# YiZhangCUG/liblcg

Measured on AMD Instinct MI355X. Metric: cg_iterations_per_sec, higher is better.
Workload: dtype f64

## Files before the change

liblcg_amd/csrc/driver.hpp:

```cpp
#pragma once

#include <algorithm>
#include <chrono>
#include <cstdlib>
#include <functional>
#include <cstring>
#include <thread>
#include <typeinfo>
#include <vector>

#include "devcommon.hpp"

namespace lcgh {

#define TRY(x) do { int rc_ = (x); if (rc_) return rc_; } while (0)
inline uintptr_t al(const void *p) { return (uintptr_t)p; }
double global_rows_of(Ctx &c, int n, const void *afp, const void *inst);

template <class Op> int launch_vec(const Op &op, long n, bool cplx, uintptr_t align_or, double *partials, hipStream_t s)
{
    const bool v2 = !cplx && (align_or & 15) == 0;
    const int g = grid_for(v2 ? (n + 1) / 2 : n);
    if (v2) hipLaunchKernelGGL((k_vec<Op, true>), dim3(g), dim3(VB), 0, s, op, n, partials);
    else hipLaunchKernelGGL((k_vec<Op, false>), dim3(g), dim3(VB), 0, s, op, n, partials);
    return g;
}

struct Driver {
    Ctx &c;
    long n;
    bool cplx;
    int max_it, abs_diff;
    double eps;
    int enq = 0;
    bool user_cb = false;

    Driver(Ctx &c_, long n_, bool cplx_, int max_it_, double eps_, int abs_diff_)
        : c(c_), n(n_), cplx(cplx_), max_it(max_it_), abs_diff(abs_diff_), eps(eps_) {}
    ~Driver() { c.in_solve = false; }
    Driver(const Driver &) = delete;

    template <class Op> int vec(Op op, uintptr_t align_or = 0) { return vec_n(op, n, align_or); }
    template <class Op> int vec_rows(Op op, int row0, uintptr_t align_or)
    {
        const PartCount keep = pcnt;
        double *table = c.partials;
        c.partials = table + (size_t)row0 * MAXG;
        int rc = vec_n(op, n, align_or);
        c.partials = table;
        const int g = pcnt.g[0];
        pcnt = keep;
        for (int r = 0; r < Op::NR; r++) pcnt.g[row0 + r] = g;
        return rc;
    }
    template <class Op> int vec_n(Op op, long n, uintptr_t align_or)
    {
        c.cnt_vec++;
        op.st = c.state;
        const int g = launch_vec(op, n, cplx, align_or, c.partials, c.stream);
        if (Op::NR > 0) pcnt.all(g);
        HIPCHK(hipGetLastError());
        return dbg(typeid(Op).name());
    }
    template <class Fin, class Op> int vecf(Fin fin, Op op, uintptr_t align_or = 0)
    {
        if (comm_active()) {
            int rc = scal(fin);
            return rc ? rc : vec(op, align_or);
        }
        c.cnt_vec++;
        const bool v2 = !cplx && (align_or & 15) == 0;
        const int g = grid_for(v2 ? (n + 1) / 2 : n);
        DevState *cur = c.state, *next = c.state == c.state_pair[0] ? c.state_pair[1] : c.state_pair[0];
        double *pin = c.partials, *pout = c.partials == c.partials_pair[0] ? c.partials_pair[1] : c.partials_pair[0];
        if (v2) hipLaunchKernelGGL((k_vecf<Fin, Op, true>), dim3(g), dim3(VB), 0, c.stream, fin, op, n, pin, pcnt, pout, cur, next);
        else hipLaunchKernelGGL((k_vecf<Fin, Op, false>), dim3(g), dim3(VB), 0, c.stream, fin, op, n, pin, pcnt, pout, cur, next);
        HIPCHK(hipGetLastError());
        c.state = next;
        if (Op::NR > 0) { c.partials = pout; pcnt.all(g); }
        return dbg(typeid(Op).name());
    }
    PartCount pcnt = [] { PartCount p; p.all(1); return p; }();
    std::function<int()> tail;
    int run_tail() { if (!tail) return 0; auto t = std::move(tail); tail = nullptr; return t(); }
    bool debug_sync = debug_level() >= 2;
    int dbg(const char *what)
    {
        if (!debug_sync) return 0;
        std::fprintf(stderr, "[lcg_hip] %s ...", what); std::fflush(stderr);
        HIPCHK(hipStreamSynchronize(c.stream));
        std::fprintf(stderr, " ok\n");
        return 0;
    }

    DevState *snap_to = nullptr;
    int snap_taken = 0;
    template <class Fin> int scal(Fin fin)
    {
        const PartCount g = pcnt;
        XgBox xb;
        c.cnt_scal++;
        if (comm_active() && Fin::NR > 0) c.cnt_allreduce++;
        if (snap_to) snap_taken++;
        if (comm_active() && Fin::NR > 0 && xg_box(&xb)) {
            hipLaunchKernelGGL((k_scal<Fin>), dim3(1), dim3(VB), 0, c.stream, fin, c.partials, g, c.state, SC_XGMI, xb, snap_to);
        } else if (comm_active() && Fin::NR > 0) {
            hipLaunchKernelGGL((k_scal<Fin>), dim3(1), dim3(VB), 0, c.stream, fin, c.partials, g, c.state, SC_REDUCE, xb, (DevState *)nullptr);
            int rc = comm_allreduce(c.state->red, Fin::NR, c.stream);
            if (rc) return rc;
            hipLaunchKernelGGL((k_scal<Fin>), dim3(1), dim3(VB), 0, c.stream, fin, c.partials, g, c.state, SC_FIN, xb, snap_to);
        } else {
            hipLaunchKernelGGL((k_scal<Fin>), dim3(1), dim3(VB), 0, c.stream, fin, c.partials, g, c.state, SC_FUSED, xb, snap_to);
        }
        HIPCHK(hipGetLastError());
        return dbg(typeid(Fin).name());
    }

    int init_state(double n_global)
    {
        c.in_solve = true; c.ax_rc = 0; c.cnt_vec = c.cnt_scal = c.cnt_allreduce = c.cnt_ax = 0;
        DevState h;
        std::memset(&h, 0, sizeof h);
        h.eps = eps; h.abs_diff = abs_diff; h.n_global = n_global; h.host = c.hstat_dev;
        h.pub_mask = comm_active() ? 0x3fffffff : ((cplx ? 2 * n : n) >= (1 << 20) ? 0 : 3);
        c.hstat->it = 0; c.hstat->done = 0; c.hstat->status = 0; c.hstat->t = 0; c.hstat->residual = 0.0;
        (void)lcg_hip_last_ax_mean_us();
        *c.state_stage = h;
        HIPCHK(hipMemcpyAsync(c.state, c.state_stage, sizeof h, hipMemcpyHostToDevice, c.stream));
        HIPCHK(hipEventRecord(c.ev_a, c.stream));
        HIPCHK(hipStreamWaitEvent(c.comm_stream, c.ev_a, 0));
        return 0;
    }
    int read_state(DevState &h)
    {
        HIPCHK(hipMemcpyAsync(&h, c.state, sizeof h, hipMemcpyDeviceToHost, c.stream));
        HIPCHK(hipStreamSynchronize(c.stream));
        return 0;
    }

    template <class F> int timed_ax(F &&call)
    {
        c.cnt_ax++;
        if (c.profile && (c.ax_seq++ % c.profile_every) == 0 && c.prof_used + 2 <= (int)c.prof_ev.size()) {
            HIPCHK(hipEventRecord(c.prof_ev[c.prof_used], c.stream));
            call();
            HIPCHK(hipEventRecord(c.prof_ev[c.prof_used + 1], c.stream));
            c.prof_used += 2;
        } else {
            call();
        }
        return c.ax_rc;
    }
    template <class F> int checked_mx(F &&call) { call(); return c.ax_rc; }

    template <class Body, class Pfp>
    int run(Body &&body, bool has_pfp, Pfp &&pfp, int code_max_it, int code_nan)
    {
        DevState h;
        int rc = 0;
        if (has_pfp || user_cb) {
            rc = read_state(h);
            if (rc) return rc;
            if (h.status == ST_ALREADY) {
                if (has_pfp) pfp(h.residual, 0);
                finish(h);
                return LCG_ALREADY_OPTIMIZIED;
            }
        }
        if (has_pfp) {
            for (;;) {
                if (pfp(h.residual, h.t)) { finish(h); return LCG_STOP; }
                if (h.residual <= eps) { finish(h); return LCG_CONVERGENCE; }
                if (max_it > 0 && h.t + 1 > max_it) { finish(h); return code_max_it; }
                rc = body(); if (rc) return rc;
                enq++;
                rc = read_state(h); if (rc) return rc;
                if (h.status == ST_COMM) return comm_lost(h);
                if (h.status == ST_NAN) { finish(h); return code_nan; }
            }
        }
        if (comm_active()) return run_lockstep(body, code_max_it, code_nan);
        const long work = cplx ? 2 * n : n;
        const int inflight = work >= (1 << 20) ? 6 : 24;
        for (;;) {
            if (max_it > 0 && enq >= max_it) break;
            rc = body(); if (rc) return rc;
            enq++;
            if (c.hstat->done) break;
            int spins = 0;
            while (c.hstat->it < enq - inflight && !c.hstat->done) {
                if (++spins > 2000) { std::this_thread::sleep_for(std::chrono::microseconds(20)); }
                if (spins > 200000) {
                    rc = read_state(h); if (rc) return rc;
                    if (h.done || h.it >= enq - inflight) break;
                    spins = 0;
                }
            }
            if ((enq & 255) == 0) {
                rc = read_state(h); if (rc) return rc;
                if (h.done) break;
            }
        }
        rc = run_tail(); if (rc) return rc;
        rc = read_state(h); if (rc) return rc;
        if (h.status == ST_COMM) return comm_lost(h);
        finish(h);
        if (h.status == ST_ALREADY) return LCG_ALREADY_OPTIMIZIED;
        if (h.status == ST_NAN) return code_nan;
        if (h.done && h.status == ST_CONVERGED) return LCG_CONVERGENCE;
        return code_max_it;
    }

    template <class Body>
    int run_lockstep(Body &&body, int code_max_it, int code_nan)
    {
        constexpr int batch = 8;
        int nb = 0, rc = 0;
        DevState h;
        for (;;) {
            int todo = batch;
            if (max_it > 0) todo = std::min(batch, max_it - enq);
            if (todo <= 0) break;
            const int slot = nb & 1;
            for (int i = 0; i < todo; i++) {
                if (i == todo - 1) { snap_to = c.snap_dev[slot]; snap_taken = 0; }
                rc = body();
                if (rc) { snap_to = nullptr; return rc; }
                enq++;
            }
            snap_to = nullptr;
            if (!snap_taken) HIPCHK(hipMemcpyAsync(c.snap[slot], c.state, sizeof(DevState), hipMemcpyDeviceToHost, c.stream));
            HIPCHK(hipEventRecord(c.snap_ev[slot], c.stream));
            nb++;
            if (nb >= 2) {
                const int prev = (nb - 2) & 1;
                HIPCHK(hipEventSynchronize(c.snap_ev[prev]));
                if (c.snap[prev]->done) break;
            }
        }
        if (nb > 0) {
            HIPCHK(hipEventSynchronize(c.snap_ev[(nb - 1) & 1]));
            HIPCHK(hipStreamSynchronize(c.stream));
            std::memcpy(&h, c.snap[(nb - 1) & 1], sizeof h);
        } else {
            rc = read_state(h); if (rc) return rc;
        }
        if (h.status == ST_COMM) return comm_lost(h);
        finish(h);
        if (h.status == ST_ALREADY) return LCG_ALREADY_OPTIMIZIED;
        if (h.status == ST_NAN) return code_nan;
        if (h.done && h.status == ST_CONVERGED) return LCG_CONVERGENCE;
        return code_max_it;
    }

    int comm_lost(const DevState &h)
    {
        finish(h);
        c.err = "direct all-reduce: a peer's contribution did not arrive in time";
        return LCG_HIP_E_COMM;
    }

    void finish(const DevState &h)
    {
        c.last_iters = h.t;
        c.last_residual = h.residual;
        c.last_ax_calls = c.prof_used / 2;
        c.last_ax_mean_us = 0.0;
        c.prof_pending = c.profile ? c.prof_used : 0;
        c.prof_used = 0;
    }
};

struct HostBridge {
    double *dm = nullptr, *dB = nullptr;
    double *hm = nullptr;
    size_t bytes = 0;
    bool active = false;
    int open(int mem, double *&m, const double *&B, size_t nbytes, hipStream_t s)
    {
        if (mem == LCG_HIP_MEM_DEVICE) return 0;
        active = true; bytes = nbytes; hm = m;
        HIPCHK(hipMalloc(&dm, nbytes));
        HIPCHK(hipMalloc(&dB, nbytes));
        HIPCHK(hipMemcpyAsync(dm, m, nbytes, hipMemcpyHostToDevice, s));
        HIPCHK(hipMemcpyAsync(dB, B, nbytes, hipMemcpyHostToDevice, s));
        m = dm; B = dB;
        return 0;
    }
    int close(hipStream_t s)
// ... 317 lines not shown
```

liblcg_amd/csrc/solvers_real.hip:

```cpp
#include <functional>

#include "driver.hpp"

namespace lcgh {

constexpr int CG1_AUTO_ROWS = 1 << 20;


struct OpDot1 {
    static constexpr int NR = 1, SKIP = SKIP_DONE;
    DevState *st; const double *a, *b;
    __device__ void prep() {}
    template <class T> __device__ void apply(long i, double *acc) { acc[0] += dotp(ld<T>(a, i), ld<T>(b, i)); }
};
struct OpDot2 {
    static constexpr int NR = 2, SKIP = SKIP_DONE;
    DevState *st; const double *a, *b;
    __device__ void prep() {}
    template <class T> __device__ void apply(long i, double *acc)
    {
        const T x = ld<T>(a, i);
        acc[0] += dotp(x, ld<T>(b, i));
        acc[1] += dotp(x, x);
    }
};

struct FinAlpha {
    static constexpr int NR = 1;
    __device__ void operator()(DevState *st, const double *sum) const
    {
        st->it++;
        if (st->done) return;
        st->s[S_AK] = st->s[S_RHO] / sum[0];
    }
};
struct FinOmega {
    static constexpr int NR = 2;
    __device__ void operator()(DevState *st, const double *sum) const
    {
        if (st->done) return;
        st->s[S_WK] = sum[0] / sum[1];
    }
};

struct FinInit {
    static constexpr int NR = 3;
    __device__ void operator()(DevState *st, const double *sum) const
    {
        const double m2 = clamp1(sum[0]), g2 = sum[1];
        st->s[S_M2] = m2; st->s[S_G2] = g2; st->s[S_RHO] = sum[2];
        double r;
        bool already = false;
        if (st->abs_diff && sqrt(g2) / st->n_global <= st->eps) { r = sqrt(g2) / st->n_global; already = true; }
        else if (g2 / m2 <= st->eps) { r = g2 / m2; already = true; }
        else r = st->abs_diff ? sqrt(g2) / st->n_global : g2 / m2;
        st->residual = r;
        if (already) { st->done = 1; st->status = ST_ALREADY; }
        publish(st);
    }
};

template <bool BICG>
struct FinClose {
    static constexpr int NR = 4;
    __device__ void operator()(DevState *st, const double *sum) const
    {
        if (!st->done) {
            st->s[S_M2] = clamp1(sum[0]);
            if (sum[3] > 0.0 || sum[0] != sum[0]) {
                st->t++;
                st->done = 1; st->status = ST_NAN;
            } else {
                const double rho_new = sum[2];
                st->s[S_BK] = BICG ? (st->s[S_AK] / st->s[S_WK]) * rho_new / st->s[S_RHO]
                                   : rho_new / st->s[S_RHO];
                st->s[S_RHO] = rho_new;
                st->s[S_G2] = sum[1];
                st->t++;
                stop_rule(st, sum[1], st->s[S_M2]);
            }
        }
        publish(st);
    }
};

struct OpZeroProbe {
    static constexpr int NR = 1, SKIP = SKIP_NEVER;
    DevState *st; const double *m;
    __device__ void prep() {}
    template <class T> __device__ void apply(long i, double *acc) { acc[0] += nonzeros(ld<T>(m, i)); }
    static __device__ double nonzeros(double v) { return v != 0.0 ? 1.0 : 0.0; }
    static __device__ double nonzeros(double2 v) { return (v.x != 0.0 ? 1.0 : 0.0) + (v.y != 0.0 ? 1.0 : 0.0); }
};
struct FinZeroGuess {
    static constexpr int NR = 1;
    __device__ void operator()(DevState *st, const double *sum) const { st->zero_guess = sum[0] == 0.0 ? 1 : 0; }
};

struct OpCgInit {
    static constexpr int NR = 3, SKIP = SKIP_NEVER;
    DevState *st; const double *Ad, *B, *m; double *g, *d;
    double *clear = nullptr;
    bool zg = false;
    __device__ void prep() { zg = st->zero_guess != 0; }
    template <class T> __device__ void apply(long i, double *acc)
    {
        const T av = ldz<T>(Ad, i, zg);
        if (zg && clear) st_(clear, i, av);
        const T gv = vsub(av, ld<T>(B, i));
        const T mv = ldz<T>(m, i, zg);
        st_(g, i, gv); st_(d, i, vneg(gv));
        acc[0] += dotp(mv, mv);
        const double gg = dotp(gv, gv);
        acc[1] += gg; acc[2] += gg;
    }
};
struct OpCgUpdate {
    static constexpr int NR = 4, SKIP = SKIP_DONE;
    DevState *st; double *m, *g; const double *d, *Ad; double ak; bool nt = false;
    __device__ void prep() { ak = st->s[S_AK]; }
    template <class T> __device__ void apply(long i, double *acc)
    {
        const T mv = vadd(ldp<T>(m, i, nt), ak * ld<T>(d, i));
        const T gv = vadd(ld<T>(g, i), ak * ldp<T>(Ad, i, nt));
        stp(m, i, mv, nt); st_(g, i, gv);
        acc[0] += dotp(mv, mv);
        const double gg = dotp(gv, gv);
        acc[1] += gg; acc[2] += gg;
        acc[3] += nanflag(mv);
    }
};
struct OpCgDir {
    static constexpr int NR = 0, SKIP = SKIP_DIR;
    DevState *st; double *d; const double *g; double bk; bool nt = false;
    __device__ void prep() { bk = st->s[S_BK]; }
    template <class T> __device__ void apply(long i, double *)
    {
        st_(d, i, vsub(bk * ld<T>(d, i), ldp<T>(g, i, nt)));
    }
};

struct OpCg1UpdateSums {
    static constexpr int NR = 4, SKIP = SKIP_DONE;
    DevState *st; double *m, *g, *d, *Ad; const double *w; double ak, bk; bool nt = false;
    __device__ void prep() { ak = st->s[S_AK]; bk = st->s[S_BK]; }
    template <class T> __device__ void apply(long i, double *acc)
    {
        const T g0 = ld<T>(g, i);
        const T dv = vsub(bk * ldp<T>(d, i, nt), g0);
        const T sv = vsub(bk * ldp<T>(Ad, i, nt), ldp<T>(w, i, nt));
        stp(d, i, dv, nt); stp(Ad, i, sv, nt);
        const T mv = vadd(ldp<T>(m, i, nt), ak * dv);
        const T gv = vadd(g0, ak * sv);
        stp(m, i, mv, nt); st_(g, i, gv);
        acc[0] += dotp(mv, mv);
        acc[1] += dotp(gv, gv);
        acc[3] += nanflag(mv);
    }
};
struct FinCg1Start {
    static constexpr int NR = 1;
    __device__ void operator()(DevState *st, const double *sum) const
    {
        if (st->done) return;
        st->s[S_AK] = st->s[S_RHO] / sum[0];
        st->s[S_BK] = 0.0;
    }
};

struct OpResidual {
    static constexpr int NR = 0, SKIP = SKIP_NEVER;
    DevState *st; const double *Ax, *B; double *r;
    double *clear = nullptr;
    bool zg = false;
    __device__ void prep() { zg = st->zero_guess != 0; }
    template <class T> __device__ void apply(long i, double *)
    {
        const T av = ldz<T>(Ax, i, zg);
        if (zg && clear) st_(clear, i, av);
        st_(r, i, vsub(ld<T>(B, i), av));
    }
};
struct OpPcgInit2 {
    static constexpr int NR = 3, SKIP = SKIP_NEVER;
    DevState *st; const double *z, *m, *r; double *d;
    __device__ void prep() {}
    template <class T> __device__ void apply(long i, double *acc)
    {
        const T zv = ld<T>(z, i), mv = ld<T>(m, i), rv = ld<T>(r, i);
        st_(d, i, zv);
        acc[0] += dotp(mv, mv); acc[1] += dotp(rv, rv); acc[2] += dotp(zv, rv);
    }
};
struct OpPcgUpdate {
    static constexpr int NR = 0, SKIP = SKIP_DONE;
    DevState *st; double *m, *r; const double *d, *Ad; double ak;
    __device__ void prep() { ak = st->s[S_AK]; }
    template <class T> __device__ void apply(long i, double *)
    {
        st_(m, i, vadd(ld<T>(m, i), ak * ld<T>(d, i)));
        st_(r, i, vsub(ld<T>(r, i), ak * ld<T>(Ad, i)));
    }
};
struct OpPcgDots {
    static constexpr int NR = 4, SKIP = SKIP_DONE;
    DevState *st; const double *m, *r, *z;
    __device__ void prep() {}
    template <class T> __device__ void apply(long i, double *acc)
    {
        const T mv = ld<T>(m, i), rv = ld<T>(r, i), zv = ld<T>(z, i);
        acc[0] += dotp(mv, mv); acc[1] += dotp(rv, rv); acc[2] += dotp(zv, rv); acc[3] += nanflag(mv);
    }
};
struct OpPcgUpdateJacobi {
    static constexpr int NR = 4, SKIP = SKIP_DONE;
    DevState *st; double *m, *r, *z; const double *d, *Ad, *invdiag; double ak; bool nt = false;
    __device__ void prep() { ak = st->s[S_AK]; }
    template <class T> __device__ void apply(long i, double *acc)
    {
        const T mv = vadd(ldp<T>(m, i, nt), ak * ld<T>(d, i));
        const T rv = vsub(ld<T>(r, i), ak * ldp<T>(Ad, i, nt));
        const T zv = vmul(ldp<T>(invdiag, i, nt), rv);
        stp(m, i, mv, nt); st_(r, i, rv); st_(z, i, zv);
        acc[0] += dotp(mv, mv); acc[1] += dotp(rv, rv); acc[2] += dotp(zv, rv); acc[3] += nanflag(mv);
    }
};
struct OpPcgDir {
    static constexpr int NR = 0, SKIP = SKIP_DIR;
    DevState *st; double *d; const double *z; double bk; bool nt = false;
    __device__ void prep() { bk = st->s[S_BK]; }
    template <class T> __device__ void apply(long i, double *) { st_(d, i, vadd(ldp<T>(z, i, nt), bk * ld<T>(d, i))); }
};

struct OpPcg1UpdateSums {
    static constexpr int NR = 5, SKIP = SKIP_DONE;
    DevState *st; double *m, *r, *z, *d, *Ad; const double *w, *invdiag; double ak, bk;
    __device__ void prep() { ak = st->s[S_AK]; bk = st->s[S_BK]; }
    template <class T> __device__ void apply(long i, double *acc)
    {
        const T dv = vadd(ld<T>(z, i), bk * ld<T>(d, i));
        const T sv = vadd(ld<T>(w, i), bk * ld<T>(Ad, i));
        st_(d, i, dv); st_(Ad, i, sv);
        const T mv = vadd(ld<T>(m, i), ak * dv);
        const T rv = vsub(ld<T>(r, i), ak * sv);
        const T zv = vmul(ld<T>(invdiag, i), rv);
        st_(m, i, mv); st_(r, i, rv); st_(z, i, zv);
        acc[0] += dotp(mv, mv); acc[1] += dotp(rv, rv); acc[2] += dotp(zv, rv); acc[3] += nanflag(mv);
    }
};
struct FinPcg1Close {
    static constexpr int NR = 5;
    __device__ void operator()(DevState *st, const double *sum) const
    {
        st->it++;
        if (!st->done) {
            st->s[S_M2] = clamp1(sum[0]);
            if (sum[3] > 0.0 || sum[0] != sum[0]) {
                st->t++;
                st->done = 1; st->status = ST_NAN;
            } else {
                const double rho_new = sum[2];
                const double bk = rho_new / st->s[S_RHO];
                st->s[S_AK] = rho_new / (sum[4] - bk * rho_new / st->s[S_AK]);
                st->s[S_BK] = bk;
                st->s[S_RHO] = rho_new;
                st->s[S_G2] = sum[1];
                st->t++;
                stop_rule(st, sum[1], st->s[S_M2]);
            }
        }
        publish(st);
    }
};

template <bool WITH_U>
struct OpShadowInit {
    static constexpr int NR = 3, SKIP = SKIP_NEVER;
    DevState *st; const double *Ax, *B, *m; double *r, *r0, *p, *u; bool zg = false;
    __device__ void prep() { zg = st->zero_guess != 0; }
    template <class T> __device__ void apply(long i, double *acc)
    {
        const T rv = vsub(ld<T>(B, i), ldz<T>(Ax, i, zg));
        const T mv = ldz<T>(m, i, zg);
        st_(r, i, rv); st_(r0, i, rv); st_(p, i, rv);
        if (WITH_U) st_(u, i, rv);
        acc[0] += dotp(mv, mv);
        const double rr = dotp(rv, rv);
        acc[1] += rr; acc[2] += rr;
    }
};
struct OpCgsQW {
    static constexpr int NR = 0, SKIP = SKIP_DONE;
    DevState *st; const double *u, *Ax; double *q, *w; double ak; bool nt = false;
    __device__ void prep() { ak = st->s[S_AK]; }
    template <class T> __device__ void apply(long i, double *)
    {
        const T uv = ld<T>(u, i);
        const T qv = vsub(uv, ak * ld<T>(Ax, i));
        st_(q, i, qv); st_(w, i, vadd(uv, qv));
    }
};
struct OpCgsUpdate {
    static constexpr int NR = 4, SKIP = SKIP_DONE;
    DevState *st; double *m, *r; const double *w, *Ax, *r0; double ak; bool nt = false;
    __device__ void prep() { ak = st->s[S_AK]; }
    template <class T> __device__ void apply(long i, double *acc)
    {
        const T mv = vadd(ldp<T>(m, i, nt), ak * ld<T>(w, i));
        const T rv = vsub(ld<T>(r, i), ak * ld<T>(Ax, i));
        stp(m, i, mv, nt); st_(r, i, rv);
        acc[0] += dotp(mv, mv); acc[1] += dotp(rv, rv); acc[2] += dotp(rv, ld<T>(r0, i)); acc[3] += nanflag(mv);
    }
};
struct OpCgsDir {
    static constexpr int NR = 0, SKIP = SKIP_DIR;
    DevState *st; double *u, *p; const double *r, *q; double bk; bool nt = false;
    __device__ void prep() { bk = st->s[S_BK]; }
    template <class T> __device__ void apply(long i, double *)
    {
        const T qv = ld<T>(q, i);
        const T uv = vadd(ld<T>(r, i), bk * qv);
        st_(u, i, uv);
        st_(p, i, vadd(uv, bk * vadd(qv, bk * ld<T>(p, i))));
    }
};
struct OpBicgS {
    static constexpr int NR = 0, SKIP = SKIP_DONE;
    DevState *st; const double *r, *Ap; double *s; double ak; bool nt = false;
    __device__ void prep() { ak = st->s[S_AK]; }
    template <class T> __device__ void apply(long i, double *) { st_(s, i, vsub(ld<T>(r, i), ak * ld<T>(Ap, i))); }
};
struct OpBicgUpdate {
    static constexpr int NR = 4, SKIP = SKIP_DONE;
    DevState *st; double *m, *r; const double *p, *s, *Ax, *r0; double ak, wk; bool nt = false;
    __device__ void prep() { ak = st->s[S_AK]; wk = st->s[S_WK]; }
    template <class T> __device__ void apply(long i, double *acc)
    {
        const T sv = ld<T>(s, i);
        const T mv = vadd(ldp<T>(m, i, nt), vadd(ak * ld<T>(p, i), wk * sv));
        const T rv = vsub(sv, wk * ld<T>(Ax, i));
        stp(m, i, mv, nt); st_(r, i, rv);
        acc[0] += dotp(mv, mv); acc[1] += dotp(rv, rv); acc[2] += dotp(rv, ld<T>(r0, i)); acc[3] += nanflag(mv);
    }
};
struct OpBicgDir {
    static constexpr int NR = 0, SKIP = SKIP_DIR;
    DevState *st; double *p; const double *r, *Ap; double bk, wk; bool nt = false;
    __device__ void prep() { bk = st->s[S_BK]; wk = st->s[S_WK]; }
    template <class T> __device__ void apply(long i, double *)
    {
        st_(p, i, vadd(ld<T>(r, i), bk * vsub(ld<T>(p, i), wk * ld<T>(Ap, i))));
    }
};


static bool stream_vectors(long n, lcg_axfunc_ptr Afp, void *inst)
{
    static const int env = [] { const char *e = std::getenv("LCG_HIP_NT_VECTORS"); return e ? atoi(e) : -1; }();
    if (env >= 0) return env != 0;
    if (n * 40L <= (128L << 20)) return false;
    if (Afp == lcg_hip_csr_ax && inst != nullptr) {
        const lcg_hip_csr *A = static_cast<const lcg_hip_csr *>(inst);
        const long nnz = A->distributed ? (long)A->loc.nnz + (long)A->rem.nnz : (long)A->main.nnz;
        return nnz * 12L >= (512L << 20);
    }
    return n * 40L > (256L << 20);
}

struct RealSolve : Solve<false> {
    using Solve::Solve;
    int ax_setup(const double *m0, double *y)
    {
        if (Afp != lcg_hip_csr_ax || inst == nullptr) return ax(m0, y);
        int rc = drv.vec(OpZeroProbe{c.state, m0}, (uintptr_t)m0);
        if (!rc) rc = drv.scal(FinZeroGuess{});
        if (rc) return rc;
        c.ax_skip = &c.state->zero_guess;
        Afp(inst, m0, y, n);
        c.ax_skip = nullptr;
        return c.ax_rc;
    }
    int ax_dot(const double *x, double *y, const double *u, bool yy, int row, bool *fused)
    {
        int f = 0, slots = 0;
        const bool builtin = Afp == lcg_hip_csr_ax && inst != nullptr;
        int rc = drv.timed_ax([&] {
            if (builtin) f = csr_ax_dot(static_cast<lcg_hip_csr *>(inst), x, y, u, yy ? 1 : 0, c.ax_partials, &slots, c.stream, &c.state->done);
            if (f == 0) Afp(inst, x, y, n);
            else if (f < 0 && !c.ax_rc) c.ax_rc = f;
        });
        *fused = f == 1;
        if (f == 1) {
            PartCount &pc = drv.pcnt;
            pc.axp = c.ax_partials; pc.ax_n = slots; pc.ax_row = row; pc.ax_yy = yy ? 1 : 0;
            pc.g[row] = 0; if (yy) pc.g[row + 1] = 0;
        }
        return rc;
    }

    bool last_body(int row)
    {
        const bool last = para.max_iterations > 0 && drv.enq + 1 >= para.max_iterations;
        if (last) { drv.pcnt.ax_n = 0; drv.pcnt.ax_row = -1; drv.pcnt.g[row] = 0; }
        return last;
    }
    template <class Close, class Op, class Rest>
    int run_self_closing(const Op &upd, uintptr_t align_or, Rest &&rest)
    {
        bool first = true;
        drv.tail = [&]() -> int { return first ? drv.scal(FinCg1Start{}) : drv.scal(Close{}); };
        const int rc = run_loop([&]() -> int {
            TRY(first ? drv.vecf(FinCg1Start{}, upd, align_or) : drv.vecf(Close{}, upd, align_or));
            first = false;
            return rest();
        });
        drv.tail = nullptr;
        return rc;
    }
};

static int check_args(const lcg_para &p, int n, const double *m, const double *B)
{
    if (n <= 0) return LCG_INVILAD_VARIABLE_SIZE;
    if (p.max_iterations < 0) return LCG_INVILAD_MAX_ITERATIONS;
    if (p.epsilon <= 0.0 || p.epsilon >= 1.0) return LCG_INVILAD_EPSILON;
    if (m == nullptr || B == nullptr) return LCG_INVALID_POINTER;
    return 0;
}

static int solve_cg(lcg_axfunc_ptr Afp, lcg_progress_ptr Pfp, double *m, const double *B, int n,
                    const lcg_para *param, void *inst, double *Gk, double *Dk, double *ADk, int mem)
{
    const lcg_para p = param ? *param : lcg_hip_default_parameters();
    TRY(check_args(p, n, m, B));
    TRY(ensure_init());
    RealSolve k(p, n, inst, Afp, Pfp);
    Ctx &c = k.c;
    TRY(k.open(mem, m, B));
    double *g, *d, *Ad;
    TRY(k.get(g, Gk)); TRY(k.get(d, Dk)); TRY(k.get(Ad, ADk));
    const bool one_reduction = c.cg_schedule == LCG_HIP_CG_ONE_REDUCTION ||
                               (c.cg_schedule == LCG_HIP_CG_AUTO && (comm_active() || (n < CG1_AUTO_ROWS && Afp == lcg_hip_csr_ax)));
    double *w = nullptr;
    if (one_reduction) TRY(k.get(w));
    if (one_reduction) TRY(k.place(B, {&w, &g, &d, &Ad}, 1));
    else TRY(k.place(B, {&Ad, &d, &g}, 1));
    TRY(k.start());
    DevState *st = c.state;
    const bool nt = stream_vectors(n, Afp, inst);

    TRY(k.ax_setup(m, Ad));
    TRY(k.drv.vec(OpCgInit{st, Ad, B, m, g, d, one_reduction ? Ad : nullptr}, al(Ad) | al(B) | al(m) | al(g) | al(d)));
    TRY(k.drv.scal(FinInit{}));
    const uintptr_t a_upd = al(m) | al(g) | al(d) | al(Ad);
    if (one_reduction) {
        bool fused; TRY(k.ax_dot(g, w, g, false, 0, &fused));
        if (!fused) TRY(k.drv.vec(OpDot1{st, g, w}, al(g) | al(w)));
        const OpCg1UpdateSums upd{st, m, g, d, Ad, w, 0.0, 0.0, nt};
        auto product = [&]() -> int {
            bool f; TRY(k.ax_dot(g, w, g, false, 2, &f));
            if (f) return 0;
            if (fused) { c.err = "A.x stopped carrying its dot in the middle of a solve"; return LCG_HIP_E_ARG; }
            return k.drv.vec_rows(OpDot1{st, g, w}, 2, al(g) | al(w));
        };
        int rc;
        if (Pfp == nullptr && !comm_active()) {
            rc = k.run_self_closing<FinCg1Close>(upd, a_upd | al(w), [&]() -> int {
                if (k.last_body(2)) return 0;
                if (fused) return product();
                TRY(k.ax(g, w));
                return k.drv.vec_rows(OpDot1{st, g, w}, 2, al(g) | al(w));
            });
        } else {
            TRY(k.drv.scal(FinCg1Start{}));
            rc = k.run_loop([&]() -> int {
                TRY(k.drv.vec(upd, a_upd | al(w)));
                if (!k.last_body(2)) TRY(product());
                return k.drv.scal(FinCg1Close{});
            });
        }
        return k.finish(rc);
    }
    int rc = k.run_loop([&]() -> int {
        bool f; TRY(k.ax_dot(d, Ad, d, false, 0, &f));
        if (!f) TRY(k.drv.vec(OpDot1{st, d, Ad}, al(d) | al(Ad)));
        TRY(k.drv.vecf(FinAlpha{}, OpCgUpdate{st, m, g, d, Ad, 0.0, nt}, a_upd));
        TRY(k.drv.vecf(FinClose<false>{}, OpCgDir{st, d, g, 0.0, nt}, al(d) | al(g)));
        return 0;
    });
    return k.finish(rc);
}

static int solve_pcg(lcg_axfunc_ptr Afp, lcg_axfunc_ptr Mfp, lcg_progress_ptr Pfp, double *m, const double *B,
                     int n, const lcg_para *param, void *inst, int mem)
{
    const lcg_para p = param ? *param : lcg_hip_default_parameters();
    TRY(check_args(p, n, m, B));
    if (Mfp == nullptr) return LCG_NULL_PRECONDITION_MATRIX;
    TRY(ensure_init());
    RealSolve k(p, n, inst, Afp, Pfp);
    Ctx &c = k.c;
    TRY(k.open(mem, m, B));
    double *r, *z, *d, *Ad;
    TRY(k.get(r)); TRY(k.get(z)); TRY(k.get(d)); TRY(k.get(Ad));
    TRY(k.place(B, {&Ad, &d, &r, &z}, 1));
    TRY(k.start());
    DevState *st = c.state;
    const bool nt = stream_vectors(n, Afp, inst);
    if (Mfp != lcg_hip_jacobi_mx) k.drv.user_cb = true;
    const double *invdiag = builtin_invdiag((const void *)Mfp, inst, n, false);

    TRY(k.ax_setup(m, Ad));
    TRY(k.drv.vec(OpResidual{st, Ad, B, r, Ad}, al(Ad) | al(B) | al(r)));
    TRY(k.drv.checked_mx([&] { Mfp(inst, r, z, n); }));
    TRY(k.drv.vec(OpPcgInit2{st, z, m, r, d}, al(z) | al(m) | al(r) | al(d)));
    TRY(k.drv.scal(FinInit{}));
    const uintptr_t a_all = al(m) | al(r) | al(z) | al(d) | al(Ad) | al(invdiag);
    const bool one_reduction = invdiag != nullptr &&
                               (c.cg_schedule == LCG_HIP_CG_ONE_REDUCTION ||
                                (c.cg_schedule == LCG_HIP_CG_AUTO && (comm_active() || (n < CG1_AUTO_ROWS && !k.drv.user_cb))));
    if (one_reduction) {
        double *w; TRY(k.get(w));
        {
            bool f; TRY(k.ax_dot(z, w, z, false, 0, &f));
            if (!f) TRY(k.drv.vec(OpDot1{st, z, w}, al(z) | al(w)));
        }
        auto product = [&]() -> int {
            bool f; TRY(k.ax_dot(z, w, z, false, 4, &f));
            if (!f) TRY(k.drv.vec_rows(OpDot1{st, z, w}, 4, al(z) | al(w)));
            return 0;
        };
        const OpPcg1UpdateSums upd{st, m, r, z, d, Ad, w, invdiag, 0.0, 0.0};
        int rc;
        if (Pfp == nullptr && !comm_active()) {
            rc = k.run_self_closing<FinPcg1Close>(upd, a_all | al(w), [&]() -> int { return k.last_body(4) ? 0 : product(); });
        } else {
            TRY(k.drv.scal(FinCg1Start{}));
            rc = k.run_loop([&]() -> int {
                TRY(k.drv.vec(upd, a_all | al(w)));
                if (!k.last_body(4)) TRY(product());
                TRY(k.drv.scal(FinPcg1Close{}));
                return 0;
            });
        }
        return k.finish(rc);
    }
    int rc = k.run_loop([&]() -> int {
        bool f; TRY(k.ax_dot(d, Ad, d, false, 0, &f));
        if (!f) TRY(k.drv.vec(OpDot1{st, d, Ad}, al(d) | al(Ad)));
        if (invdiag) {
            TRY(k.drv.vecf(FinAlpha{}, OpPcgUpdateJacobi{st, m, r, z, d, Ad, invdiag, 0.0, nt}, a_all));
        } else {
            TRY(k.drv.vecf(FinAlpha{}, OpPcgUpdate{st, m, r, d, Ad, 0.0}, a_all));
            TRY(k.drv.checked_mx([&] { Mfp(inst, r, z, n); }));
            TRY(k.drv.vec(OpPcgDots{st, m, r, z}, a_all));
        }
        TRY(k.drv.vecf(FinClose<false>{}, OpPcgDir{st, d, z, 0.0, nt && invdiag != nullptr}, al(d) | al(z)));
        return 0;
    });
    return k.finish(rc);
}

static int solve_cgs(lcg_axfunc_ptr Afp, lcg_progress_ptr Pfp, double *m, const double *B, int n,
                     const lcg_para *param, void *inst, double *RK, double *R0T, double *PK, double *AX,
                     double *UK, double *QK, double *WK, int mem)
{
    const lcg_para p = param ? *param : lcg_hip_default_parameters();
    TRY(check_args(p, n, m, B));
    TRY(ensure_init());
    RealSolve k(p, n, inst, Afp, Pfp);
    TRY(k.open(mem, m, B));
    double *r, *r0, *pk, *Ax, *u, *q, *w;
    TRY(k.get(r, RK)); TRY(k.get(r0, R0T)); TRY(k.get(pk, PK)); TRY(k.get(Ax, AX));
    TRY(k.get(u, UK)); TRY(k.get(q, QK)); TRY(k.get(w, WK));
    TRY(k.place(B, {&Ax, &pk, &w, &u, &q, &r, &r0}, 1));
    TRY(k.start());
    DevState *st = k.c.state;
    const bool nt = stream_vectors(n, Afp, inst);
    const uintptr_t a_all = al(m) | al(B) | al(r) | al(r0) | al(pk) | al(Ax) | al(u) | al(q) | al(w);

    TRY(k.ax_setup(m, Ax));
    TRY(k.drv.vec(OpShadowInit<true>{st, Ax, B, m, r, r0, pk, u}, a_all));
    TRY(k.drv.scal(FinInit{}));
    int rc = k.run_loop([&]() -> int {
        bool f; TRY(k.ax_dot(pk, Ax, r0, false, 0, &f));
        if (!f) TRY(k.drv.vec(OpDot1{st, Ax, r0}, a_all));
        TRY(k.drv.vecf(FinAlpha{}, OpCgsQW{st, u, Ax, q, w, 0.0, nt}, a_all));
        TRY(k.ax(w, Ax));
        TRY(k.drv.vec(OpCgsUpdate{st, m, r, w, Ax, r0, 0.0, nt}, a_all));
        TRY(k.drv.vecf(FinClose<false>{}, OpCgsDir{st, u, pk, r, q, 0.0, nt}, a_all));
        return 0;
    });
    return k.finish(rc);
}

static int solve_bicgstab(lcg_axfunc_ptr Afp, lcg_progress_ptr Pfp, double *m, const double *B, int n,
                          const lcg_para *param, void *inst, int mem)
{
    const lcg_para p = param ? *param : lcg_hip_default_parameters();
    TRY(check_args(p, n, m, B));
    TRY(ensure_init());
    RealSolve k(p, n, inst, Afp, Pfp);
    TRY(k.open(mem, m, B));
    double *r, *r0, *pk, *Ax, *s, *Ap;
    TRY(k.get(r)); TRY(k.get(r0)); TRY(k.get(pk)); TRY(k.get(Ax)); TRY(k.get(s)); TRY(k.get(Ap));
    TRY(k.place(B, {&Ap, &Ax, &pk, &s, &r, &r0}, 2));
    TRY(k.start());
    DevState *st = k.c.state;
    const bool nt = stream_vectors(n, Afp, inst);
    const uintptr_t a_all = al(m) | al(B) | al(r) | al(r0) | al(pk) | al(Ax) | al(s) | al(Ap);

    TRY(k.ax_setup(m, Ax));
    TRY(k.drv.vec(OpShadowInit<false>{st, Ax, B, m, r, r0, pk, nullptr}, a_all));
    TRY(k.drv.scal(FinInit{}));
    int rc = k.run_loop([&]() -> int {
        bool f; TRY(k.ax_dot(pk, Ap, r0, false, 0, &f));
        if (!f) TRY(k.drv.vec(OpDot1{st, Ap, r0}, a_all));
        TRY(k.drv.vecf(FinAlpha{}, OpBicgS{st, r, Ap, s, 0.0, nt}, a_all));
        TRY(k.ax_dot(s, Ax, s, true, 0, &f));
        if (!f) TRY(k.drv.vec(OpDot2{st, Ax, s}, a_all));
        TRY(k.drv.vecf(FinOmega{}, OpBicgUpdate{st, m, r, pk, s, Ax, r0, 0.0, 0.0, nt}, a_all));
        TRY(k.drv.vecf(FinClose<true>{}, OpBicgDir{st, pk, r, Ap, 0.0, 0.0, nt}, a_all));
        return 0;
    });
    return k.finish(rc);
}

enum { S_RESTART = 8, S_MID = 9 };

struct OpBicgS2 {
    static constexpr int NR = 1, SKIP = SKIP_DONE;
    DevState *st; const double *r, *Ap; double *s; double ak;
    __device__ void prep() { ak = st->s[S_AK]; }
    template <class T> __device__ void apply(long i, double *acc)
    {
        const T sv = vsub(ld<T>(r, i), ak * ld<T>(Ap, i));
        st_(s, i, sv);
        acc[0] += dotp(sv, sv);
    }
};
struct FinMid {
    static constexpr int NR = 1;
    int abs_diff;
    __device__ void operator()(DevState *st, const double *sum) const
    {
        if (!abs_diff) return;
        if (!st->done) {
            st->t++;
            const double res = sqrt(sum[0]) / st->n_global;
            st->residual = res;
            if (res <= st->eps) { st->done = 1; st->status = ST_CONVERGED; st->s[S_MID] = 1.0; }
        }
        publish(st);
    }
};
struct OpMidFinish {
    static constexpr int NR = 1, SKIP = SKIP_NEVER;
    DevState *st; double *m; const double *p; double ak; bool active;
    __device__ void prep() { active = st->s[S_MID] == 1.0; ak = st->s[S_AK]; }
    template <class T> __device__ void apply(long i, double *acc)
    {
        if (!active) return;
        const T mv = vadd(ld<T>(m, i), ak * ld<T>(p, i));
        st_(m, i, mv);
        acc[0] += nanflag(mv);
    }
};
struct FinMidNan {
    static constexpr int NR = 1;
    __device__ void operator()(DevState *st, const double *sum) const
    {
        if (st->s[S_MID] != 1.0) return;
        st->s[S_MID] = 2.0;
        if (sum[0] > 0.0) st->status = ST_NAN;
        publish(st);
    }
};
struct FinOmega2 {
    static constexpr int NR = 2;
    int counts_body;
    __device__ void operator()(DevState *st, const double *sum) const
    {
        if (counts_body) st->it++;
        if (st->done) return;
        st->s[S_WK] = sum[0] / sum[1];
    }
};
struct FinClose2 {
    static constexpr int NR = 4;
    double restart_eps;
    __device__ void operator()(DevState *st, const double *sum) const
    {
        if (!st->done) {
            st->s[S_M2] = clamp1(sum[0]);
            if (sum[3] > 0.0 || sum[0] != sum[0]) { st->t++; st->done = 1; st->status = ST_NAN; }
            else {
                const double rho_new = sum[2];
                if (fabs(rho_new) < restart_eps) {
                    st->s[S_RESTART] = 1.0;
                    st->s[S_RHO] = sum[1];
                } else {
                    st->s[S_RESTART] = 0.0;
                    st->s[S_BK] = (st->s[S_AK] / st->s[S_WK]) * rho_new / st->s[S_RHO];
                    st->s[S_RHO] = rho_new;
                }
                st->s[S_G2] = sum[1];
                st->t++;
                stop_rule(st, sum[1], st->s[S_M2]);
            }
        }
        publish(st);
    }
};
struct OpBicgDir2 {
    static constexpr int NR = 0, SKIP = SKIP_DIR;
    DevState *st; double *p, *r0; const double *r, *Ap; double bk, wk; bool restart;
    __device__ void prep() { bk = st->s[S_BK]; wk = st->s[S_WK]; restart = st->s[S_RESTART] != 0.0; }
    template <class T> __device__ void apply(long i, double *)
    {
        const T rv = ld<T>(r, i);
        if (restart) { st_(r0, i, rv); st_(p, i, rv); }
        else st_(p, i, vadd(rv, bk * vsub(ld<T>(p, i), wk * ld<T>(Ap, i))));
    }
};

static int solve_bicgstab2(lcg_axfunc_ptr Afp, lcg_progress_ptr Pfp, double *m, const double *B, int n,
                           const lcg_para *param, void *inst, int mem)
{
    const lcg_para p = param ? *param : lcg_hip_default_parameters();
    if (n <= 0) return LCG_INVILAD_VARIABLE_SIZE;
    if (p.max_iterations < 0) return LCG_INVILAD_MAX_ITERATIONS;
    if (p.epsilon <= 0.0) return LCG_INVILAD_EPSILON;
    if (p.restart_epsilon <= 0.0 || p.epsilon >= 1.0) return LCG_INVILAD_RESTART_EPSILON;
    if (m == nullptr || B == nullptr) return LCG_INVALID_POINTER;
    TRY(ensure_init());
    RealSolve k(p, n, inst, Afp, Pfp);
    TRY(k.open(mem, m, B));
    double *r, *r0, *pk, *Ax, *s, *Ap;
    TRY(k.get(r)); TRY(k.get(r0)); TRY(k.get(pk)); TRY(k.get(Ax)); TRY(k.get(s)); TRY(k.get(Ap));
    TRY(k.place(B, {&Ap, &Ax, &pk, &s, &r, &r0}, 2));
    TRY(k.start());
    DevState *st = k.c.state;
    const uintptr_t a_all = al(m) | al(B) | al(r) | al(r0) | al(pk) | al(Ax) | al(s) | al(Ap);
    const int halves = p.abs_diff ? 1 : 0;

    TRY(k.ax(m, Ax));
    TRY(k.drv.vec(OpShadowInit<false>{st, Ax, B, m, r, r0, pk, nullptr}, a_all));
    TRY(k.drv.scal(FinInit{}));
    auto first_half = [&]() -> int {
        TRY(k.ax(pk, Ap));
        TRY(k.drv.vec(OpDot1{st, Ap, r0}, a_all));
        TRY(k.drv.scal(FinAlpha{}));
        TRY(k.drv.vec(OpBicgS2{st, r, Ap, s, 0.0}, a_all));
        TRY(k.drv.scal(FinMid{halves}));
        if (halves) {
            TRY(k.drv.vec(OpMidFinish{st, m, pk, 0.0, false}, a_all));
            TRY(k.drv.scal(FinMidNan{}));
        }
        return 0;
    };
// ... 63 lines not shown
```

Baseline: 1536.

## Trim solve setup and teardown launches, fold init reduction into first update

Several per-solve fixed costs are cut. The zero-guess probe becomes a single kernel that clears a preset flag, replacing a reduction plus scalar kernel. In the one-reduction CG/PCG path the init scalar kernel is folded into the first update's finalizer. On a capped last iteration the final direction update is skipped and the state is snapshotted directly. The cross-stream event is dropped when no comm is active, and the final state read goes through a snapshot buffer and an event sync. This adds control-flow complexity around the first and last iterations and changes the partial-row bookkeeping.

```diff
diff --git a/liblcg_amd/csrc/driver.hpp b/liblcg_amd/csrc/driver.hpp
--- a/liblcg_amd/csrc/driver.hpp
+++ b/liblcg_amd/csrc/driver.hpp
@@ -34,6 +34,7 @@
     double eps;
     int enq = 0;
     bool user_cb = false;
+    bool guess_probed = false;
 
     Driver(Ctx &c_, long n_, bool cplx_, int max_it_, double eps_, int abs_diff_)
         : c(c_), n(n_), cplx(cplx_), max_it(max_it_), abs_diff(abs_diff_), eps(eps_) {}
@@ -95,6 +96,15 @@
 
     DevState *snap_to = nullptr;
     int snap_taken = 0;
+    bool state_in_snap = false;
+    template <class Fin> int scal_last(Fin fin)
+    {
+        snap_to = c.snap_dev[0];
+        const int rc = scal(fin);
+        snap_to = nullptr;
+        state_in_snap = rc == 0;
+        return rc;
+    }
     template <class Fin> int scal(Fin fin)
     {
         const PartCount g = pcnt;
@@ -122,19 +132,25 @@
         DevState h;
         std::memset(&h, 0, sizeof h);
         h.eps = eps; h.abs_diff = abs_diff; h.n_global = n_global; h.host = c.hstat_dev;
+        h.zero_guess = guess_probed ? 1 : 0;
         h.pub_mask = comm_active() ? 0x3fffffff : ((cplx ? 2 * n : n) >= (1 << 20) ? 0 : 3);
         c.hstat->it = 0; c.hstat->done = 0; c.hstat->status = 0; c.hstat->t = 0; c.hstat->residual = 0.0;
         (void)lcg_hip_last_ax_mean_us();
         *c.state_stage = h;
         HIPCHK(hipMemcpyAsync(c.state, c.state_stage, sizeof h, hipMemcpyHostToDevice, c.stream));
-        HIPCHK(hipEventRecord(c.ev_a, c.stream));
-        HIPCHK(hipStreamWaitEvent(c.comm_stream, c.ev_a, 0));
+        if (comm_active()) {
+            HIPCHK(hipEventRecord(c.ev_a, c.stream));
+            HIPCHK(hipStreamWaitEvent(c.comm_stream, c.ev_a, 0));
+        }
         return 0;
     }
     int read_state(DevState &h)
     {
-        HIPCHK(hipMemcpyAsync(&h, c.state, sizeof h, hipMemcpyDeviceToHost, c.stream));
-        HIPCHK(hipStreamSynchronize(c.stream));
+        if (!state_in_snap) HIPCHK(hipMemcpyAsync(c.snap[0], c.state, sizeof h, hipMemcpyDeviceToHost, c.stream));
+        state_in_snap = false;
+        HIPCHK(hipEventRecord(c.snap_ev[0], c.stream));
+        HIPCHK(hipEventSynchronize(c.snap_ev[0]));
+        std::memcpy(&h, c.snap[0], sizeof h);
         return 0;
     }
 
diff --git a/liblcg_amd/csrc/solvers_real.hip b/liblcg_amd/csrc/solvers_real.hip
--- a/liblcg_amd/csrc/solvers_real.hip
+++ b/liblcg_amd/csrc/solvers_real.hip
@@ -92,6 +92,21 @@
     static __device__ double nonzeros(double v) { return v != 0.0 ? 1.0 : 0.0; }
     static __device__ double nonzeros(double2 v) { return (v.x != 0.0 ? 1.0 : 0.0) + (v.y != 0.0 ? 1.0 : 0.0); }
 };
+template <bool VEC2>
+__global__ __launch_bounds__(VB) void k_zero_probe(const double *m, long n, DevState *st)
+{
+    const long stride = (long)gridDim.x * VB;
+    const long tid = (long)blockIdx.x * VB + threadIdx.x;
+    double nz = 0.0;
+    if (VEC2) {
+        const long n2 = n >> 1;
+        for (long i = tid; i < n2; i += stride) nz += OpZeroProbe::nonzeros(ld<double2>(m, i));
+        if ((n & 1) && tid == 0) nz += OpZeroProbe::nonzeros(ld<double>(m, n - 1));
+    } else {
+        for (long i = tid; i < n; i += stride) nz += OpZeroProbe::nonzeros(ld<double>(m, i));
+    }
+    if (__syncthreads_or(nz != 0.0) && threadIdx.x == 0) st->zero_guess = 0;
+}
 struct FinZeroGuess {
     static constexpr int NR = 1;
     __device__ void operator()(DevState *st, const double *sum) const { st->zero_guess = sum[0] == 0.0 ? 1 : 0; }
@@ -164,6 +179,16 @@
     {
         if (st->done) return;
         st->s[S_AK] = st->s[S_RHO] / sum[0];
+        st->s[S_BK] = 0.0;
+    }
+};
+struct FinInitStart {
+    static constexpr int NR = 4;
+    __device__ void operator()(DevState *st, const double *sum) const
+    {
+        FinInit{}(st, sum);
+        if (st->done) return;
+        st->s[S_AK] = st->s[S_RHO] / sum[3];
         st->s[S_BK] = 0.0;
     }
 };
@@ -372,9 +397,19 @@
     int ax_setup(const double *m0, double *y)
     {
         if (Afp != lcg_hip_csr_ax || inst == nullptr) return ax(m0, y);
-        int rc = drv.vec(OpZeroProbe{c.state, m0}, (uintptr_t)m0);
-        if (!rc) rc = drv.scal(FinZeroGuess{});
-        if (rc) return rc;
+        if (drv.guess_probed) {
+            const bool v2 = (al(m0) & 15) == 0;
+            const int g = grid_for(v2 ? ((long)n + 1) / 2 : (long)n);
+            c.cnt_vec++;
+            if (v2) hipLaunchKernelGGL((k_zero_probe<true>), dim3(g), dim3(VB), 0, c.stream, m0, (long)n, c.state);
+            else hipLaunchKernelGGL((k_zero_probe<false>), dim3(g), dim3(VB), 0, c.stream, m0, (long)n, c.state);
+            HIPCHK(hipGetLastError());
+            TRY(drv.dbg("k_zero_probe"));
+        } else {
+            int rc = drv.vec(OpZeroProbe{c.state, m0}, (uintptr_t)m0);
+            if (!rc) rc = drv.scal(FinZeroGuess{});
+            if (rc) return rc;
+        }
         c.ax_skip = &c.state->zero_guess;
         Afp(inst, m0, y, n);
         c.ax_skip = nullptr;
@@ -398,19 +433,30 @@
         return rc;
     }
 
+    int start_probing()
+    {
+        drv.guess_probed = Afp == lcg_hip_csr_ax && inst != nullptr && !comm_active();
+        return start();
+    }
+
     bool last_body(int row)
     {
         const bool last = para.max_iterations > 0 && drv.enq + 1 >= para.max_iterations;
         if (last) { drv.pcnt.ax_n = 0; drv.pcnt.ax_row = -1; drv.pcnt.g[row] = 0; }
         return last;
     }
+    bool last_capped_body() const
+    {
+        return para.max_iterations > 0 && drv.enq + 1 >= para.max_iterations && Afp == lcg_hip_csr_ax && inst != nullptr && Pfp == nullptr && !comm_active();
+    }
+    bool init_rides(bool one_reduction) const { return one_reduction && Pfp == nullptr && !comm_active() && !drv.user_cb; }
     template <class Close, class Op, class Rest>
-    int run_self_closing(const Op &upd, uintptr_t align_or, Rest &&rest)
+    int run_self_closing(const Op &upd, uintptr_t align_or, bool init_rides, Rest &&rest)
     {
         bool first = true;
-        drv.tail = [&]() -> int { return first ? drv.scal(FinCg1Start{}) : drv.scal(Close{}); };
+        drv.tail = [&]() -> int { return !first ? drv.scal_last(Close{}) : init_rides ? drv.scal_last(FinInitStart{}) : drv.scal_last(FinCg1Start{}); };
         const int rc = run_loop([&]() -> int {
-            TRY(first ? drv.vecf(FinCg1Start{}, upd, align_or) : drv.vecf(Close{}, upd, align_or));
+            TRY(!first ? drv.vecf(Close{}, upd, align_or) : init_rides ? drv.vecf(FinInitStart{}, upd, align_or) : drv.vecf(FinCg1Start{}, upd, align_or));
             first = false;
             return rest();
         });
@@ -445,17 +491,18 @@
     if (one_reduction) TRY(k.get(w));
     if (one_reduction) TRY(k.place(B, {&w, &g, &d, &Ad}, 1));
     else TRY(k.place(B, {&Ad, &d, &g}, 1));
-    TRY(k.start());
+    TRY(k.start_probing());
     DevState *st = c.state;
     const bool nt = stream_vectors(n, Afp, inst);
 
     TRY(k.ax_setup(m, Ad));
     TRY(k.drv.vec(OpCgInit{st, Ad, B, m, g, d, one_reduction ? Ad : nullptr}, al(Ad) | al(B) | al(m) | al(g) | al(d)));
-    TRY(k.drv.scal(FinInit{}));
+    const bool ride = k.init_rides(one_reduction);
+    if (!ride) TRY(k.drv.scal(FinInit{}));
     const uintptr_t a_upd = al(m) | al(g) | al(d) | al(Ad);
     if (one_reduction) {
-        bool fused; TRY(k.ax_dot(g, w, g, false, 0, &fused));
-        if (!fused) TRY(k.drv.vec(OpDot1{st, g, w}, al(g) | al(w)));
+        bool fused; TRY(k.ax_dot(g, w, g, false, ride ? 3 : 0, &fused));
+        if (!fused) TRY(ride ? k.drv.vec_rows(OpDot1{st, g, w}, 3, al(g) | al(w)) : k.drv.vec(OpDot1{st, g, w}, al(g) | al(w)));
         const OpCg1UpdateSums upd{st, m, g, d, Ad, w, 0.0, 0.0, nt};
         auto product = [&]() -> int {
             bool f; TRY(k.ax_dot(g, w, g, false, 2, &f));
@@ -465,7 +512,7 @@
         };
         int rc;
         if (Pfp == nullptr && !comm_active()) {
-            rc = k.run_self_closing<FinCg1Close>(upd, a_upd | al(w), [&]() -> int {
+            rc = k.run_self_closing<FinCg1Close>(upd, a_upd | al(w), ride, [&]() -> int {
                 if (k.last_body(2)) return 0;
                 if (fused) return product();
                 TRY(k.ax(g, w));
@@ -485,6 +532,7 @@
         bool f; TRY(k.ax_dot(d, Ad, d, false, 0, &f));
         if (!f) TRY(k.drv.vec(OpDot1{st, d, Ad}, al(d) | al(Ad)));
         TRY(k.drv.vecf(FinAlpha{}, OpCgUpdate{st, m, g, d, Ad, 0.0, nt}, a_upd));
+        if (Dk == nullptr && k.last_capped_body()) return k.drv.scal_last(FinClose<false>{});
         TRY(k.drv.vecf(FinClose<false>{}, OpCgDir{st, d, g, 0.0, nt}, al(d) | al(g)));
         return 0;
     });
@@ -504,7 +552,7 @@
     double *r, *z, *d, *Ad;
     TRY(k.get(r)); TRY(k.get(z)); TRY(k.get(d)); TRY(k.get(Ad));
     TRY(k.place(B, {&Ad, &d, &r, &z}, 1));
-    TRY(k.start());
+    TRY(k.start_probing());
     DevState *st = c.state;
     const bool nt = stream_vectors(n, Afp, inst);
     if (Mfp != lcg_hip_jacobi_mx) k.drv.user_cb = true;
@@ -514,16 +562,17 @@
     TRY(k.drv.vec(OpResidual{st, Ad, B, r, Ad}, al(Ad) | al(B) | al(r)));
     TRY(k.drv.checked_mx([&] { Mfp(inst, r, z, n); }));
     TRY(k.drv.vec(OpPcgInit2{st, z, m, r, d}, al(z) | al(m) | al(r) | al(d)));
-    TRY(k.drv.scal(FinInit{}));
     const uintptr_t a_all = al(m) | al(r) | al(z) | al(d) | al(Ad) | al(invdiag);
     const bool one_reduction = invdiag != nullptr &&
                                (c.cg_schedule == LCG_HIP_CG_ONE_REDUCTION ||
                                 (c.cg_schedule == LCG_HIP_CG_AUTO && (comm_active() || (n < CG1_AUTO_ROWS && !k.drv.user_cb))));
+    const bool ride = k.init_rides(one_reduction);
+    if (!ride) TRY(k.drv.scal(FinInit{}));
     if (one_reduction) {
         double *w; TRY(k.get(w));
         {
-            bool f; TRY(k.ax_dot(z, w, z, false, 0, &f));
-            if (!f) TRY(k.drv.vec(OpDot1{st, z, w}, al(z) | al(w)));
+            bool f; TRY(k.ax_dot(z, w, z, false, ride ? 3 : 0, &f));
+            if (!f) TRY(ride ? k.drv.vec_rows(OpDot1{st, z, w}, 3, al(z) | al(w)) : k.drv.vec(OpDot1{st, z, w}, al(z) | al(w)));
         }
         auto product = [&]() -> int {
             bool f; TRY(k.ax_dot(z, w, z, false, 4, &f));
@@ -533,7 +582,7 @@
         const OpPcg1UpdateSums upd{st, m, r, z, d, Ad, w, invdiag, 0.0, 0.0};
         int rc;
         if (Pfp == nullptr && !comm_active()) {
-            rc = k.run_self_closing<FinPcg1Close>(upd, a_all | al(w), [&]() -> int { return k.last_body(4) ? 0 : product(); });
+            rc = k.run_self_closing<FinPcg1Close>(upd, a_all | al(w), ride, [&]() -> int { return k.last_body(4) ? 0 : product(); });
         } else {
             TRY(k.drv.scal(FinCg1Start{}));
             rc = k.run_loop([&]() -> int {
@@ -555,6 +604,7 @@
             TRY(k.drv.checked_mx([&] { Mfp(inst, r, z, n); }));
             TRY(k.drv.vec(OpPcgDots{st, m, r, z}, a_all));
         }
+        if (k.last_capped_body()) return k.drv.scal_last(FinClose<false>{});
         TRY(k.drv.vecf(FinClose<false>{}, OpPcgDir{st, d, z, 0.0, nt && invdiag != nullptr}, al(d) | al(z)));
         return 0;
     });
@@ -574,7 +624,7 @@
     TRY(k.get(r, RK)); TRY(k.get(r0, R0T)); TRY(k.get(pk, PK)); TRY(k.get(Ax, AX));
     TRY(k.get(u, UK)); TRY(k.get(q, QK)); TRY(k.get(w, WK));
     TRY(k.place(B, {&Ax, &pk, &w, &u, &q, &r, &r0}, 1));
-    TRY(k.start());
+    TRY(k.start_probing());
     DevState *st = k.c.state;
     const bool nt = stream_vectors(n, Afp, inst);
     const uintptr_t a_all = al(m) | al(B) | al(r) | al(r0) | al(pk) | al(Ax) | al(u) | al(q) | al(w);
@@ -605,7 +655,7 @@
     double *r, *r0, *pk, *Ax, *s, *Ap;
     TRY(k.get(r)); TRY(k.get(r0)); TRY(k.get(pk)); TRY(k.get(Ax)); TRY(k.get(s)); TRY(k.get(Ap));
     TRY(k.place(B, {&Ap, &Ax, &pk, &s, &r, &r0}, 2));
-    TRY(k.start());
+    TRY(k.start_probing());
     DevState *st = k.c.state;
     const bool nt = stream_vectors(n, Afp, inst);
     const uintptr_t a_all = al(m) | al(B) | al(r) | al(r0) | al(pk) | al(Ax) | al(s) | al(Ap);
```

Measured after the change: 1533, median of 2. About the same (-0.2%).
